# BurntSushi/aho-corasick

Measured on NVIDIA H100. Metric: haystack_scan_throughput, higher is better.
Workload: dtype u8

## Files before the change

aho-corasick_b200/csrc/acb_prefilter.cu:

```cuda
#include "acb_device.cuh"
#ifndef ACB_PTX_HEADER
#define ACB_PTX_HEADER "acb_ptx.cuh"
#endif
#include ACB_PTX_HEADER

#include <cstdio>
#include <cstdlib>
#include <type_traits>

#include <cub/device/device_scan.cuh>
#include <cub/device/device_select.cuh>

namespace acb {
namespace {

enum : int { kGeomNarrow = 0, kGeomWide = 1 };
template <int GEOM> struct PfGeom {
  static constexpr int kThreads = GEOM == kGeomNarrow ? 1024 : 512;
  static constexpr int kWarps = kThreads / 32;
  static constexpr int kGroups = GEOM == kGeomNarrow ? 2 : 4;
  static constexpr int kTile = kGroups * 512;
  static constexpr int kStageBytes = kTile + 16;
  static constexpr int kMinCtas = GEOM == kGeomWide ? 2 : 1;
};
template <bool DENSE> struct PfCfg {
  static constexpr int kSlots = 256;
  static constexpr int kQ2 = DENSE ? 64 : 96;
};

__device__ __forceinline__ uint32_t bloom_hash2(uint32_t x) {
  x ^= x >> 16;
  x *= 0x7feb352du;
  x ^= x >> 15;
  x *= 0x846ca68bu;
  x ^= x >> 16;
  return x;
}

__device__ __forceinline__ uint32_t bloom_hash3(uint32_t x) {
  x ^= x >> 15;
  x *= 0x2c1b3c6du;
  x ^= x >> 12;
  x *= 0x297a2d39u;
  x ^= x >> 15;
  return x;
}

#ifdef ACB_EMULATE
static const uint32_t kWinShift = getenv("ACB_EMU_WINSHIFT") ? (uint32_t)atoi(getenv("ACB_EMU_WINSHIFT")) : 31u;
#else
constexpr uint32_t kWinShift = 31;
#endif

constexpr int kPfStages = 2;

struct Emitter {
  uint64_t* g_keys;
  uint32_t* g_pids;
  unsigned long long* g_counter;
  uint64_t cap;
  __device__ __forceinline__ void emit(uint64_t key, uint32_t pid) {
    const unsigned m = __activemask();
    const int leader = __ffs(m) - 1;
    const int lane = threadIdx.x & 31;
    unsigned long long base = 0;
    if (lane == leader) base = atomicAdd(g_counter, (unsigned long long)__popc(m));
    base = __shfl_sync(m, base, leader);
    const unsigned long long g = base + __popc(m & ((1u << lane) - 1));
    if (g < cap) { g_keys[g] = key; g_pids[g] = pid; }
  }
};

__device__ __forceinline__ uint32_t anchor_lookup(const DfaDev& d, const PrefilterLaunch& p, uint64_t s) {
  if (s + d.amap_k > p.span_end) return 0;
  const uintptr_t a = reinterpret_cast<uintptr_t>(p.hay + s);
  const uintptr_t lo_edge = reinterpret_cast<uintptr_t>(p.hay), hi_edge = lo_edge + p.hay_len;
  const uintptr_t wa = a & ~uintptr_t(3);
  uint32_t key;
  if (wa >= lo_edge && wa + ((a & 3) ? 8 : 4) <= hi_edge) {
    const uint32_t* w = reinterpret_cast<const uint32_t*>(wa);
    const uint32_t lo = __ldg(w);
    const uint32_t hi = (a & 3) ? __ldg(w + 1) : 0u;
    key = __funnelshift_r(lo, hi, (uint32_t)(a & 3) * 8) & d.amap_kmask;
  } else {
    key = 0;
    for (uint32_t i = 0; i < d.amap_k; ++i) key |= (uint32_t)__ldg(p.hay + s + i) << (8 * i);
  }
  uint32_t slot = bloom_hash3(key) >> d.amap_shift;
  for (;;) {
    const uint2 e = __ldg(d.amap + slot);
    if (e.y == 0 || e.x == key) return e.y;
    slot = (slot + 1) & d.amap_mask;
  }
}

__device__ __forceinline__ uint32_t anchor_lookup_key(const DfaDev& d, uint32_t key) {
  uint32_t slot = bloom_hash3(key) >> d.amap_shift;
  for (;;) {
    const uint2 e = __ldg(d.amap + slot);
    if (e.y == 0 || e.x == key) return e.y;
    slot = (slot + 1) & d.amap_mask;
  }
}

template <int MODE>
__device__ __forceinline__ void verify_from(const DfaDev& d, const PrefilterLaunch& p, const uint8_t* s_cls,
                                            uint64_t s, uint32_t sid, uint32_t j, Emitter& em) {
  const uint8_t* __restrict__ hay = p.hay;
  const uint32_t* __restrict__ trans = d.trans;
  uint64_t pos = s + j;
  uint32_t best_pid = 0, best_len = 0;
  bool entered = j != 0;
  for (;;) {
    if (!entered) {
      if (pos >= p.span_end) break;
      const uint32_t b = __ldg(hay + pos);
      sid = __ldg(trans + sid + s_cls[b]);
      ++j;
      ++pos;
      if (sid == 0) break;
      if (__ldg(d.depth16 + (sid >> d.stride2)) != j) break;
    }
    entered = false;
    if (sid <= d.max_match_id) {
      const uint32_t row = sid >> d.stride2;
      const uint32_t lo = __ldg(d.match_offsets + row - 2), hi = __ldg(d.match_offsets + row - 1);
      if (MODE == 0) {
        for (uint32_t i = lo; i < hi; ++i) {
          const uint32_t pid = __ldg(d.match_pids + i);
          if (__ldg(d.pattern_lens + pid) != j) break;
          if (p.first_only && i > lo) break;
          const uint64_t tie = ((uint64_t)(d.max_pattern_len - j) << p.dup_shift) | (uint64_t)(i - lo);
          em.emit(((pos - p.span_start) << kTieBits) | tie, pid);
        }
      } else {
        const uint32_t pid = __ldg(d.match_pids + lo);
        if (__ldg(d.pattern_lens + pid) == j) { best_pid = pid; best_len = j; }
      }
    }
  }
  if (MODE == 1 && best_len) em.emit(((s - p.span_start) << kTieBits) | best_len, best_pid);
}

template <int MODE>
__device__ __forceinline__ void verify_at(const DfaDev& d, const PrefilterLaunch& p, const uint8_t* s_cls,
                                          uint64_t s, Emitter& em) {
  if (d.amap != nullptr) {
    const uint32_t sid = anchor_lookup(d, p, s);
    if (sid != 0) verify_from<MODE>(d, p, s_cls, s, sid, d.amap_k, em);
  } else {
    verify_from<MODE>(d, p, s_cls, s, d.start_unanchored_id, 0, em);
  }
}

template <int GEOM> struct PfBloom {
  static constexpr uint32_t kLogBits = GEOM == kGeomWide ? 17 : 20;
  static constexpr uint32_t kShift = 35 - kLogBits;
};

template <uint32_t SHIFT>
__device__ __forceinline__ bool bloom_test(const uint32_t* s_bitmap, uint32_t h) {
  const uint32_t byte = reinterpret_cast<const uint8_t*>(s_bitmap)[h >> SHIFT];
  const uint32_t rep = byte * 0x01010101u;
  return (__funnelshift_r(rep, rep, h) & 1u) != 0;
}

template <int MODE, bool MASKED, bool DENSE, int STRIDE, int GEOM, int DYN = 0>
__global__ void __launch_bounds__(PfGeom<GEOM>::kThreads, PfGeom<GEOM>::kMinCtas)
prefilter_kernel(DfaDev d, PrefilterLaunch p) {
  static_assert(STRIDE == 1 || STRIDE == 2, "fingerprint stride");
  static_assert(GEOM == kGeomNarrow || STRIDE == 2, "the 2 KiB tile needs the stride-2 first stage (32 hit bits per lane)");
  constexpr bool ANCH = DENSE;
  constexpr int kPfThreads = PfGeom<GEOM>::kThreads;
  constexpr int kPfWarps = PfGeom<GEOM>::kWarps;
  constexpr int kPfTile = PfGeom<GEOM>::kTile;
  constexpr int kPfStageBytes = PfGeom<GEOM>::kStageBytes;
  constexpr int kGroups = PfGeom<GEOM>::kGroups;
  constexpr int kPfSlots = PfCfg<DENSE>::kSlots;
  constexpr int kSlotsAlloc = kPfSlots;
  constexpr int kPfQ2 = PfCfg<ANCH>::kQ2;
  constexpr uint32_t kBloomShift = PfBloom<GEOM>::kShift;
  using Q2Entry = typename std::conditional<ANCH, uint2, uint32_t>::type;
  ACB_DYNAMIC_SMEM(smem_raw);
  unsigned char* s_ring = smem_raw;
  uint64_t* s_bars = reinterpret_cast<uint64_t*>(s_ring + kPfWarps * kPfStages * kPfStageBytes);
  uint32_t* s_tile_of = reinterpret_cast<uint32_t*>(s_bars + kPfWarps * kPfStages);
  uint32_t* s_next_tile = s_tile_of + kPfWarps * kPfStages;
  Q2Entry* s_queue2 = reinterpret_cast<Q2Entry*>(s_next_tile + 4);
  uint16_t* s_slots = reinterpret_cast<uint16_t*>(s_queue2 + kPfWarps * kPfQ2);
  uint32_t* s_bitmap = reinterpret_cast<uint32_t*>(s_slots + kPfWarps * kSlotsAlloc);
  __shared__ uint8_t s_cls[256];

  const int tid = threadIdx.x;
  const int lane = tid & 31;
  const int warp = tid >> 5;
  const uint32_t bitmap_words = p.brute ? 0u : (1u << (p.log_bits - 5));
  for (uint32_t i = tid; i < bitmap_words; i += kPfThreads) s_bitmap[i] = p.bitmap[i];
  if (tid < 256) s_cls[tid] = d.classes[tid];
  if (tid < kPfWarps * kPfStages) ptx::mbar_init(ptx::smem_addr(&s_bars[tid]), 1);
  if (tid == 0) {
    *reinterpret_cast<uint64_t*>(s_next_tile) = DYN == 2 ? (uint64_t)blockIdx.x << 32 : 0ull;
    s_next_tile[2] = 0xFFFFFFFEu;
  }
  ptx::mbar_init_fence();
  ptx::fence_proxy_async();
  __syncthreads();

  Emitter em{p.keys, p.pids, p.counter, p.cap};
  unsigned long long cand_total = 0;

  if (blockIdx.x == 0) {
    const uint64_t tail_lo = (p.region_hi > p.region_lo && !p.brute) ? p.region_hi - (STRIDE - 1) : p.region_hi;
    const uint64_t head_n = p.region_lo - p.scan_lo;
    const uint64_t tail_n = p.scan_hi > tail_lo ? p.scan_hi - tail_lo : 0;
    for (uint64_t i = tid; i < head_n + tail_n; i += kPfThreads) {
      const uint64_t s = i < head_n ? p.scan_lo + i : tail_lo + (i - head_n);
      verify_at<MODE>(d, p, s_cls, s, em);
    }
  }

  const uint64_t n_blocks16 = (p.region_hi - p.region_lo) >> 4;
  const uint64_t per_cta = (n_blocks16 + gridDim.x - 1) / gridDim.x;
  const uint64_t b0 = (uint64_t)blockIdx.x * per_cta;
  const uint64_t b1 = min(b0 + per_cta, n_blocks16);
  const uint64_t split_lo = p.region_lo + (b0 << 4);
  const uint64_t split_hi = b0 < b1 ? p.region_lo + (b1 << 4) : split_lo;

  if (p.brute) {
    for (uint64_t s = split_lo + tid; s < split_hi; s += kPfThreads) verify_at<MODE>(d, p, s_cls, s, em);
    if (tid == 0 && split_hi > split_lo) atomicAdd(p.counter + 1, (unsigned long long)(split_hi - split_lo));
    return;
  }
  constexpr bool whole = DYN == 2;
  const uint64_t chunk_lo = whole ? p.region_lo : split_lo;
  const uint64_t chunk_hi = whole ? p.region_hi : split_hi;

  const uint32_t kmask = p.kmask, fold = p.fold, mult = p.mult;
  const uint32_t fold1 = p.fold & 0x00FFFFFFu;
  const uint32_t mult8 = p.mult3 << p.key_shift;
  const uint64_t chunk_base = chunk_lo - (uint64_t)(STRIDE - 1);
  const uint32_t rel_bias = (uint32_t)(STRIDE - 1);
  const uint8_t* s_bytes = reinterpret_cast<const uint8_t*>(s_bitmap);
  unsigned char* ring = s_ring + warp * (kPfStages * kPfStageBytes);
  uint64_t* bars = s_bars + warp * kPfStages;
  uint16_t* slots = s_slots + warp * kSlotsAlloc;
  Q2Entry* q2 = s_queue2 + warp * kPfQ2;
  uint32_t q2len = 0;
  uint32_t q2win = 0;

  auto drain2 = [&]() {
    __syncwarp();
    const uint64_t win_base = chunk_base + ((uint64_t)q2win << kWinShift);
    for (uint32_t i = lane; i < q2len; i += 32) {
      if constexpr (ANCH) {
        const uint2 e = q2[i];
        if (e.y != 0) verify_from<MODE>(d, p, s_cls, win_base + e.x, e.y, d.amap_k, em);
        else verify_at<MODE>(d, p, s_cls, win_base + e.x, em);
      } else {
        verify_at<MODE>(d, p, s_cls, win_base + q2[i], em);
      }
    }
    cand_total += q2len;
    q2len = 0;
    __syncwarp();
  };

  const uint64_t chunk_bytes = chunk_hi - chunk_lo;
  const uint32_t n_tiles = (uint32_t)((chunk_bytes + kPfTile - 1) / kPfTile);
  const uint32_t last_valid = n_tiles ? (uint32_t)(chunk_bytes - (uint64_t)(n_tiles - 1) * kPfTile) : 0;
  const bool use_windows = (chunk_bytes >> kWinShift) != 0;
  uint32_t bar0 = ptx::smem_addr(bars), ring0 = ptx::smem_addr(ring), lane0 = ring0 + (uint32_t)lane * 16u;
  ptx::keep_in_registers(bar0, ring0, lane0);
  const uint8_t* chunk_src = p.hay + chunk_lo;
  auto issue = [&](uint32_t t, uint32_t stage) {
    const uint32_t bytes = (t + 1 < n_tiles ? (uint32_t)kPfTile : last_valid) + 16;
    const uint32_t bar = bar0 + stage * 8, dst = ring0 + stage * kPfStageBytes;
    ptx::mbar_arrive_expect_tx(bar, bytes);
    ptx::tma_load_1d(dst, chunk_src + (uint64_t)t * kPfTile, bytes, bar);
  };
  constexpr uint32_t kDrawBatch = 4, kSuper = 256;
  static_assert(kSuper % (2 * kDrawBatch) == 0, "batches never straddle a super-tile or its half-way mark");
  uint32_t* tile_of = s_tile_of + warp * kPfStages;
  const uint32_t draw_a = ptx::smem_addr(s_next_tile), next_a = draw_a + 8;
  const uint32_t n_super = (n_tiles + kSuper - 1) / kSuper;
  constexpr uint64_t kNoMore = 0xFFFFFFFFull << 32;
  constexpr uint32_t kUnpublished = 0xFFFFFFFEu, kNone = 0xFFFFFFFFu;
  uint32_t batch_next = 0, batch_left = 0;
  bool exhausted = false;
  unsigned long long pend_g = 0;
  bool have_pend = false;
  auto publish = [&]() {
    if (have_pend) {
      ptx::sts32_volatile(next_a, pend_g < n_super ? (uint32_t)pend_g : kNone);
      have_pend = false;
    }
  };
  auto draw = [&](uint32_t stage) {
    if constexpr (DYN == 1) {
      if (batch_left == 0) {
        batch_next = ptx::atoms_add(draw_a, kDrawBatch);
        batch_left = kDrawBatch;
      }
      const uint32_t t = batch_next++;
      --batch_left;
      tile_of[stage] = t;
      if (t < n_tiles) issue(t, stage);
      return;
    }
    publish();
    while (batch_left == 0 && !exhausted) {
      const uint64_t v = ptx::atoms_add64(draw_a, kDrawBatch);
      const uint32_t sup = (uint32_t)(v >> 32), off = (uint32_t)v;
      if (sup == kNone) { exhausted = true; break; }
      if (off == kSuper / 2) { pend_g = atomicAdd(p.counter + 2, 1ull) + gridDim.x; have_pend = true; }
      if (off < kSuper) { batch_next = sup * kSuper + off; batch_left = kDrawBatch; break; }
      if (off == kSuper) {
        uint32_t g;
        while ((g = ptx::lds32_volatile(next_a)) == kUnpublished) {}
        ptx::sts32_volatile(next_a, kUnpublished);
        if (g != kNone) {
          ptx::atoms_exch64(draw_a, ((uint64_t)g << 32) | kDrawBatch);
          batch_next = g * kSuper;
          batch_left = kDrawBatch;
        } else {
          ptx::atoms_exch64(draw_a, kNoMore);
          exhausted = true;
        }
        break;
      }
      while ((uint32_t)(ptx::lds64_volatile(draw_a) >> 32) == sup) {}
    }
    uint32_t t = n_tiles;
    if (!exhausted) { t = batch_next++; --batch_left; }
    tile_of[stage] = t;
    if (t < n_tiles) issue(t, stage);
  };
  if (lane == 0) {
    if constexpr (DYN) {
      draw(0);
      draw(1);
    } else {
      if ((uint32_t)warp < n_tiles) issue((uint32_t)warp, 0);
      if ((uint32_t)warp + kPfWarps < n_tiles) issue((uint32_t)warp + kPfWarps, 1);
    }
  }
  __syncwarp();
  constexpr int kBitsPerGroup = 16 / STRIDE;
  constexpr int kHitBits = kGroups * kBitsPerGroup;
  for (uint32_t it = 0;; ++it) {
    const uint32_t stage = it & 1;
    const uint32_t parity = (it >> 1) & 1;
    uint32_t t;
    if constexpr (DYN) t = *reinterpret_cast<volatile uint32_t*>(tile_of + stage);
    else t = (uint32_t)warp + it * (uint32_t)kPfWarps;
    if (t >= n_tiles) break;
    const uint64_t wbase = chunk_lo + (uint64_t)t * kPfTile;
    uint32_t win = 0;
    if (use_windows) {
      win = (uint32_t)(((uint64_t)t * kPfTile) >> kWinShift);
      if (win != q2win) {
        if (q2len) drain2();
        q2win = win;
      }
    }
    while (!ptx::mbar_try_wait(bar0 + stage * 8, parity)) {}
    const uint32_t stage_off = stage * (uint32_t)kPfStageBytes;
    const uint32_t tile_a = ring0 + stage_off;
    uint32_t wv[kGroups][5];
#pragma unroll
    for (int g = 0; g < kGroups; ++g) {
      const uint32_t ga = lane0 + stage_off + g * 512;
      const uint4 v = ptx::lds128(ga);
      wv[g][0] = v.x; wv[g][1] = v.y; wv[g][2] = v.z; wv[g][3] = v.w;
      wv[g][4] = ptx::lds32(ga + 16);
    }
    uint32_t mask = 0;
#define ACB_WIN(o, lo, hi) (((o) & 3) ? __funnelshift_r(lo, hi, ((o) & 3) * 8) : (lo))
#define ACB_PROBE(o, lo, hi)                                                                  \
  do {                                                                                        \
    uint32_t gm, h, sel;                                                                      \
    if constexpr (STRIDE == 2) {                                                              \
      gm = MASKED ? (ACB_WIN(o, lo, hi) | fold1) : ACB_WIN(o, lo, hi);                        \
      h = gm * mult8;                                                                         \
      sel = gm;                                                                               \
    } else {                                                                                  \
      gm = MASKED ? ((ACB_WIN(o, lo, hi) | fold) & kmask) : ACB_WIN(o, lo, hi);               \
      h = gm * mult;                                                                          \
      sel = h;                                                                                \
    }                                                                                         \
    if constexpr (DENSE) {                                                                    \
                        \
      const uint32_t ph = __umulhi(gm, mult);                                                  \
      const uint32_t bw = s_bitmap[h >> (kBloomShift + 2)];                                    \
      mask = __funnelshift_r(mask, __funnelshift_r(bw, bw, ph) & __funnelshift_r(bw, bw, ph >> 5), 1); \
    } else {                                                                                  \
      const uint32_t rep = (uint32_t)s_bytes[h >> kBloomShift] * 0x01010101u;                 \
      mask = __funnelshift_r(mask, __funnelshift_r(rep, rep, sel), 1);                        \
    }                                                                                         \
  } while (0)
#pragma unroll
    for (int g = 0; g < kGroups; ++g) {
#pragma unroll
      for (int wi = 0; wi < 4; ++wi) {
        if constexpr (STRIDE == 1) {
          ACB_PROBE(0, wv[g][wi], wv[g][wi + 1]); ACB_PROBE(1, wv[g][wi], wv[g][wi + 1]);
          ACB_PROBE(2, wv[g][wi], wv[g][wi + 1]); ACB_PROBE(3, wv[g][wi], wv[g][wi + 1]);
        } else {
          ACB_PROBE(0, wv[g][wi], wv[g][wi + 1]); ACB_PROBE(2, wv[g][wi], wv[g][wi + 1]);
        }
      }
    }
#undef ACB_PROBE
#undef ACB_WIN
    if constexpr (kHitBits < 32) mask >>= (32 - kHitBits);
    if (t + 1 == n_tiles) {
      uint32_t ok_bits = 0;
#pragma unroll
      for (int g = 0; g < kGroups; ++g)
        if ((uint32_t)(g * 512 + lane * 16) < last_valid) ok_bits |= (uint32_t)((1ull << kBitsPerGroup) - 1) << (g * kBitsPerGroup);
      mask &= ok_bits;
    }
    auto hit_offset = [&](uint32_t b, uint32_t ln) -> uint32_t {
      return (b / kBitsPerGroup) * 512 + ln * 16 + (b % kBitsPerGroup) * STRIDE;
    };
    const uint32_t cnt = __popc(mask);
    const uint32_t lt = (1u << lane) - 1;
    constexpr int kPlanes = DENSE ? 4 : 3;
    uint32_t slot = 0, total = 0;
    constexpr int kSumPlanes = kPlanes;
#pragma unroll
    for (int b = 0; b < kSumPlanes; ++b) {
      const uint32_t bl = __ballot_sync(0xffffffffu, (cnt >> b) & 1u);
      slot += __popc(bl & lt) << b;
      total += __popc(bl) << b;
    }
    if (__any_sync(0xffffffffu, (cnt >> kPlanes) != 0)) total = (uint32_t)kPfSlots + 1;
    if (total) {
      const bool region_first = (whole || blockIdx.x == 0) && t == 0;
      if (total > (uint32_t)kPfSlots) {
        uint32_t nver = 0;
        while (mask) {
          const int b = __ffs(mask) - 1;
          mask &= mask - 1;
          const uint64_t e = wbase + hit_offset((uint32_t)b, (uint32_t)lane);
#pragma unroll
          for (int j = 0; j < STRIDE; ++j)
            if (e >= p.region_lo + j) { verify_at<MODE>(d, p, s_cls, e - j, em); ++nver; }
        }
        cand_total += __reduce_add_sync(0xffffffffu, nver);
      } else {
        {
          uint16_t* sp = slots + slot;
          const uint32_t tag = (uint32_t)lane << 5;
          while (mask) {
            const uint32_t b = (uint32_t)__ffs(mask) - 1;
            mask &= mask - 1;
            *sp++ = (uint16_t)(tag | b);
          }
        }
        __syncwarp();
        const uint32_t wrel = (use_windows ? (uint32_t)((wbase - chunk_lo) - ((uint64_t)win << kWinShift)) : (uint32_t)(wbase - chunk_lo)) + rel_bias;
        const uint32_t n_items = total * STRIDE;
        if constexpr (ANCH) {
          for (uint32_t base = 0; base < n_items; base += 64) {
            uint32_t rel2[2], key2[2], slot2[2], sid2[2];
            bool look[2], pass2[2];
            uint2 ent[2];
#pragma unroll
            for (int u = 0; u < 2; ++u) {
              const uint32_t w = base + 32u * u + lane;
              const uint32_t j = STRIDE == 2 ? (w & 1u) : 0u;
              look[u] = false; pass2[u] = false; rel2[u] = 0; key2[u] = 0; slot2[u] = 0; sid2[u] = 0;
              ent[u] = make_uint2(0, 0);
              if (w < n_items) {
                const uint32_t raw = slots[STRIDE == 2 ? (w >> 1) : w];
                const uint32_t e = hit_offset(raw & 31u, raw >> 5);
                rel2[u] = wrel + e - j;
                if (STRIDE == 2 && e < j) {
                  pass2[u] = !region_first;
                } else if (d.amap == nullptr) {
                  pass2[u] = true;
                } else if (chunk_base + ((uint64_t)win << kWinShift) + rel2[u] + d.amap_k <= p.span_end) {
                  const uint32_t off = e - j;
                  const uint32_t sa = tile_a + (off & ~3u);
                  key2[u] = __funnelshift_r(ptx::lds32(sa), ptx::lds32(sa + 4), (off & 3) * 8) & d.amap_kmask;
                  slot2[u] = bloom_hash3(key2[u]) >> d.amap_shift;
                  look[u] = true;
                }
              }
            }
#pragma unroll
            for (int u = 0; u < 2; ++u)
              if (look[u]) ent[u] = __ldg(d.amap + slot2[u]);
#pragma unroll
            for (int u = 0; u < 2; ++u) {
              if (look[u]) {
                while (ent[u].y != 0 && ent[u].x != key2[u]) {
                  slot2[u] = (slot2[u] + 1) & d.amap_mask;
                  ent[u] = __ldg(d.amap + slot2[u]);
                }
                sid2[u] = ent[u].y;
                pass2[u] = sid2[u] != 0;
              }
              const uint32_t bal = __ballot_sync(0xffffffffu, pass2[u]);
              if (bal) {
                if (pass2[u]) q2[q2len + __popc(bal & lt)] = make_uint2(rel2[u], sid2[u]);
                q2len += __popc(bal);
                if (q2len > (uint32_t)(kPfQ2 - 32)) drain2();
              }
            }
          }
        } else
        for (uint32_t base = 0; base < n_items; base += 32) {
          const uint32_t w = base + lane;
          const uint32_t j = STRIDE == 2 ? (w & 1u) : 0u;
          bool pass = false;
          uint32_t gram_keep = 0, e = 0;
          if (w < n_items) {
            const uint32_t raw = slots[STRIDE == 2 ? (w >> 1) : w];
            e = hit_offset(raw & 31u, raw >> 5);
            if (STRIDE == 2 && e < j) {
              pass = !region_first;
            } else {
              const uint32_t off = e - j;
              const uint32_t sa = tile_a + (off & ~3u);
              uint32_t gram = __funnelshift_r(ptx::lds32(sa), ptx::lds32(sa + 4), (off & 3) * 8);
              if (MASKED) gram = (gram | fold) & kmask;
              if (STRIDE == 2) pass = bloom_test<kBloomShift>(s_bitmap, gram * mult) && bloom_test<kBloomShift>(s_bitmap, bloom_hash2(gram));
              else pass = bloom_test<kBloomShift>(s_bitmap, bloom_hash2(gram));
            }
          }
          const uint32_t bal = __ballot_sync(0xffffffffu, pass);
          if (bal) {
            if (pass) {
              const uint32_t rel = wrel + e - j;
              if constexpr (!ANCH) q2[q2len + __popc(bal & lt)] = rel;
            }
            q2len += __popc(bal);
            if (q2len > (uint32_t)(kPfQ2 - 32)) drain2();
          }
        }
      }
    }
    __syncwarp();
    if (lane == 0) {
      if constexpr (DYN) draw(stage);
      else if (t + 2 * kPfWarps < n_tiles) issue(t + 2 * kPfWarps, stage);
    }
  }
  if constexpr (DYN == 2) { if (lane == 0) publish(); }
  if (q2len) drain2();
  if (lane == 0 && cand_total) atomicAdd(p.counter + 1, cand_total);
}

constexpr int kBsThreads = 512;
constexpr int kBsWarps = kBsThreads / 32;
constexpr int kBsQueue = 128;

template <int MODE>
__global__ void __launch_bounds__(kBsThreads, 2) bytescan_kernel(DfaDev d, PrefilterLaunch p) {
  __shared__ uint8_t s_cls[256];
  __shared__ uint64_t s_q[kBsWarps * kBsQueue];
  const int tid = threadIdx.x, lane = tid & 31, warp = tid >> 5;
  if (tid < 256) s_cls[tid] = d.classes[tid];
  __syncthreads();
  Emitter em{p.keys, p.pids, p.counter, p.cap};
  unsigned long long cand_total = 0;
  if (blockIdx.x == 0) {
    const uint64_t head_n = p.region_lo - p.scan_lo;
    const uint64_t tail_n = p.scan_hi > p.region_hi ? p.scan_hi - p.region_hi : 0;
    for (uint64_t i = tid; i < head_n + tail_n; i += kBsThreads)
      verify_at<MODE>(d, p, s_cls, i < head_n ? p.scan_lo + i : p.region_hi + (i - head_n), em);
  }
  uint64_t* q = s_q + warp * kBsQueue;
  uint32_t qlen = 0;
  auto drain = [&]() {
    __syncwarp();
    for (uint32_t i = lane; i < qlen; i += 32) verify_at<MODE>(d, p, s_cls, q[i], em);
    cand_total += qlen;
    qlen = 0;
    __syncwarp();
  };
  const uint32_t n_needles = p.bs_n;
  const uint32_t max_back = max(p.bs_back[0], max(p.bs_back[1], p.bs_back[2]));
  const uint32_t owned_lanes = max_back ? 31u : 32u;
  const uint64_t step_bytes = (uint64_t)owned_lanes * 16;
  const uint64_t region_bytes = p.region_hi - p.region_lo;
  const uint64_t n_steps = (region_bytes + step_bytes - 1) / step_bytes;
  const uint32_t lt = (1u << lane) - 1;
  const uint64_t load_end = p.region_hi + (max_back ? 16 : 0);
  auto load = [&](uint64_t base) -> uint4 {
    return base < load_end ? ptx::ld_nc_u4(p.hay + base) : make_uint4(0, 0, 0, 0);
  };
  auto process = [&](uint64_t base, const uint4& v) {
    const bool in_range = base < load_end;
    const uint32_t w[4] = {v.x, v.y, v.z, v.w};
    uint32_t zany = 0;
#pragma unroll
    for (int j = 0; j < 3; ++j) {
      if (j >= (int)n_needles) break;
      const uint32_t needle = p.bs_needle[j];
#pragma unroll
      for (int k = 0; k < 4; ++k) {
        const uint32_t x = w[k] ^ needle;
        zany |= (x - 0x01010101u) & ~x & 0x80808080u;
      }
    }
    if (!__any_sync(0xffffffffu, zany != 0 && in_range)) return;
    uint32_t cand = 0;
#pragma unroll
    for (int j = 0; j < 3; ++j) {
      if (j >= (int)n_needles) break;
      const uint32_t needle = p.bs_needle[j];
      uint32_t m = 0;
#pragma unroll
      for (int k = 0; k < 4; ++k) {
        const uint32_t x = w[k] ^ needle;
        const uint32_t z = (x - 0x01010101u) & ~x & 0x80808080u;
        m |= ((((z >> 7) * 0x00204081u) >> 21) & 0xFu) << (4 * k);
      }
      if (!in_range) m = 0;
      const uint32_t back = p.bs_back[j];
      if (back == 0) {
        cand |= m;
      } else {
        const uint32_t both = m | (__shfl_down_sync(0xffffffffu, m, 1) << 16);
        uint32_t smear = both;
        for (uint32_t sft = 1; sft <= back; ++sft) smear |= both >> sft;
        cand |= smear & 0xFFFFu;
      }
    }
    if (lane >= (int)owned_lanes || base >= p.region_hi) cand = 0;
    const uint32_t cnt = __popc(cand);
    if (__any_sync(0xffffffffu, cnt != 0)) {
      uint32_t slot = 0, total = 0;
#pragma unroll
      for (int b = 0; b < 5; ++b) {
        const uint32_t bl = __ballot_sync(0xffffffffu, (cnt >> b) & 1u);
        slot += __popc(bl & lt) << b;
        total += __popc(bl) << b;
      }
      if (qlen + total > (uint32_t)kBsQueue) drain();
      if (total > (uint32_t)kBsQueue) {
        uint32_t c = cand, nver = 0;
        while (c) {
          const int bit = __ffs(c) - 1;
          c &= c - 1;
          verify_at<MODE>(d, p, s_cls, base + bit, em);
          ++nver;
        }
        cand_total += __reduce_add_sync(0xffffffffu, nver);
      } else {
        uint64_t* dst = q + qlen + slot;
        uint32_t c = cand;
        while (c) {
          const int bit = __ffs(c) - 1;
          c &= c - 1;
          *dst++ = base + bit;
        }
        qlen += total;
        if (qlen >= 64) drain();
      }
    }
  };
  const uint64_t stride = (uint64_t)gridDim.x * kBsWarps;
  auto base_of = [&](uint64_t st) { return p.region_lo + st * step_bytes + (uint64_t)lane * 16; };
  uint64_t st = (uint64_t)blockIdx.x * kBsWarps + warp;
  uint4 cur[2], nxt[2];
#pragma unroll
  for (int u = 0; u < 2; ++u) cur[u] = st + u * stride < n_steps ? load(base_of(st + u * stride)) : make_uint4(0, 0, 0, 0);
  for (; st < n_steps; st += 2 * stride) {
#pragma unroll
    for (int u = 0; u < 2; ++u) {
      const uint64_t sn = st + (2 + u) * stride;
      nxt[u] = sn < n_steps ? load(base_of(sn)) : make_uint4(0, 0, 0, 0);
    }
#pragma unroll
    for (int u = 0; u < 2; ++u)
      if (st + u * stride < n_steps) process(base_of(st + u * stride), cur[u]);
    cur[0] = nxt[0];
    cur[1] = nxt[1];
  }
  if (qlen) drain();
  if (lane == 0 && cand_total) atomicAdd(p.counter + 1, cand_total);
}


__device__ __forceinline__ void tuple_span(const ChainLaunch& c, uint64_t i, uint64_t* s, uint64_t* e) {
  const uint64_t key = c.keys[i];
  if (c.mode == 1) {
    *s = key >> kTieBits;
    *e = *s + (key & kTieMask);
  } else {
    *e = key >> kTieBits;
    *s = *e - c.pattern_lens[c.pids[i]];
  }
}

__global__ void chain_ends_kernel(ChainLaunch c) {
  const uint64_t i = (uint64_t)blockIdx.x * blockDim.x + threadIdx.x;
  if (i >= c.n) return;
  uint64_t s, e;
  tuple_span(c, i, &s, &e);
  c.scratch_end[i] = e;
}

__global__ void chain_select_kernel(ChainLaunch c) {
  const uint64_t i = (uint64_t)blockIdx.x * blockDim.x + threadIdx.x;
  if (i >= c.n) return;
  uint64_t s, e;
  tuple_span(c, i, &s, &e);
  if (i > 0 && c.scratch_end[i - 1] > s) return;
  c.flags[i] = 1;
  uint64_t cur_end = e;
  for (uint64_t j = i + 1; j < c.n; ++j) {
    uint64_t sj, ej;
    tuple_span(c, j, &sj, &ej);
    if (c.scratch_end[j - 1] <= sj) break;
    if (sj >= cur_end) { c.flags[j] = 1; cur_end = ej; } else c.flags[j] = 0;
  }
}

struct MaxOp {
  __device__ __forceinline__ uint64_t operator()(uint64_t a, uint64_t b) const { return a > b ? a : b; }
};

}

cudaError_t launch_prefilter(const DfaDev& dfa, const PrefilterLaunch& p, int sm_count, cudaStream_t s) {
  const bool dense = p.dense != 0;
  const int geom = p.stride == 2 ? p.geom : kGeomNarrow;
  if (geom < kGeomNarrow || geom > kGeomWide) return cudaErrorInvalidValue;
  const uint32_t want_log = geom == kGeomWide ? PfBloom<kGeomWide>::kLogBits : PfBloom<kGeomNarrow>::kLogBits;
  if (!p.brute && (p.log_bits != want_log || p.shift != 35 - want_log)) return cudaErrorInvalidValue;
  const size_t bitmap_bytes = p.brute ? 0 : (size_t(1) << (p.log_bits - 3));
  static const int kThreadsOf[2] = {PfGeom<0>::kThreads, PfGeom<1>::kThreads};
  static const int kStageOf[2] = {PfGeom<0>::kStageBytes, PfGeom<1>::kStageBytes};
  static const int kTileOf[2] = {PfGeom<0>::kTile, PfGeom<1>::kTile};
  const int threads = kThreadsOf[geom];
  const int warps = threads / 32;
  const int stage_bytes = kStageOf[geom];
  const int tile = kTileOf[geom];
  const int q2_bytes = dense ? PfCfg<true>::kQ2 * 8 : PfCfg<false>::kQ2 * 4;
  const int slot_bytes = PfCfg<false>::kSlots * 2;
  const size_t smem = size_t(warps) * (kPfStages * stage_bytes + kPfStages * 12 + q2_bytes + slot_bytes) + 16 + bitmap_bytes;
  if (smem > 227 * 1024 - 1024) return cudaErrorInvalidValue;
  const bool masked = p.fold != 0 || p.kmask != 0xFFFFFFFFu;
  using KernT = void (*)(DfaDev, PrefilterLaunch);
#define ACB_PF_ROW(M, K, D)                                                                                 \
  {prefilter_kernel<M, K, false, 1, kGeomNarrow, D>, prefilter_kernel<M, K, true, 1, kGeomNarrow, D>, \
   prefilter_kernel<M, K, false, 2, kGeomNarrow, D>, prefilter_kernel<M, K, false, 2, kGeomWide, D>}
  static const KernT table[2][2][3][4] = {
      {{ACB_PF_ROW(0, false, 0), ACB_PF_ROW(0, false, 1), ACB_PF_ROW(0, false, 2)},
       {ACB_PF_ROW(0, true, 0), ACB_PF_ROW(0, true, 1), ACB_PF_ROW(0, true, 2)}},
      {{ACB_PF_ROW(1, false, 0), ACB_PF_ROW(1, false, 1), ACB_PF_ROW(1, false, 2)},
       {ACB_PF_ROW(1, true, 0), ACB_PF_ROW(1, true, 1), ACB_PF_ROW(1, true, 2)}}};
#undef ACB_PF_ROW
  if (p.dyn > 2) return cudaErrorInvalidValue;
  if (p.stride == 2 && dense) return cudaErrorInvalidValue;
  int variant = dense ? 1 : 0;
  if (p.stride == 2) variant = geom == kGeomWide ? 3 : 2;
  KernT kern = table[p.mode ? 1 : 0][masked ? 1 : 0][p.dyn][variant];
#ifdef ACB_EMULATE
  if (getenv("ACB_EMU_TRACE")) fprintf(stderr, "launch_prefilter variant %d dyn %d threads %d smem %zu\n", variant, (int)p.dyn, threads, smem);
#endif
  cudaError_t e = cudaFuncSetAttribute(kern, cudaFuncAttributeMaxDynamicSharedMemorySize, (int)smem);
  if (e != cudaSuccess) return e;
  int per_sm = 1;
  e = cudaOccupancyMaxActiveBlocksPerMultiprocessor(&per_sm, kern, threads, smem);
  if (e != cudaSuccess) return e;
  if (per_sm < 1) per_sm = 1;
  uint64_t grid = (uint64_t)sm_count * per_sm;
  const uint64_t cta_step = uint64_t(warps) * tile;
  const uint64_t warp_steps = ((p.region_hi - p.region_lo) + cta_step - 1) / cta_step;
  if (grid > warp_steps) grid = warp_steps ? warp_steps : 1;
  ACB_LAUNCH(kern, (unsigned)grid, threads, smem, s, dfa, p);
  return cudaGetLastError();
}

cudaError_t launch_bytescan(const DfaDev& dfa, const PrefilterLaunch& p, int sm_count, cudaStream_t s) {
  if (p.bs_n < 1 || p.bs_n > 3) return cudaErrorInvalidValue;
  for (uint32_t j = 0; j < 3; ++j)
    if (p.bs_back[j] > 15) return cudaErrorInvalidValue;
  uint64_t grid = (uint64_t)sm_count * 2;
  const uint64_t steps = ((p.region_hi - p.region_lo) + 16 * 31 - 1) / (16 * 31);
  const uint64_t ctas = (steps + kBsWarps - 1) / kBsWarps;
  if (grid > ctas) grid = ctas ? ctas : 1;
  if (p.mode) ACB_LAUNCH(bytescan_kernel<1>, (unsigned)grid, kBsThreads, 0, s, dfa, p);
  else ACB_LAUNCH(bytescan_kernel<0>, (unsigned)grid, kBsThreads, 0, s, dfa, p);
  return cudaGetLastError();
}

cudaError_t launch_chain_ends(const ChainLaunch& c, cudaStream_t s) {
  const unsigned blocks = (unsigned)((c.n + 255) / 256);
  ACB_LAUNCH(chain_ends_kernel, blocks, 256, 0, s, c);
  return cudaGetLastError();
}
cudaError_t launch_chain_select(const ChainLaunch& c, cudaStream_t s) {
  const unsigned blocks = (unsigned)((c.n + 255) / 256);
  ACB_LAUNCH(chain_select_kernel, blocks, 256, 0, s, c);
  return cudaGetLastError();
}
cudaError_t scan_max_u64(void* d_temp, size_t& temp_bytes, uint64_t* data, uint64_t n, cudaStream_t s) {
  return cub::DeviceScan::InclusiveScan(d_temp, temp_bytes, data, data, MaxOp(), (int64_t)n, s);
}
cudaError_t select_flagged(void* d_temp, size_t& temp_bytes, const uint64_t* keys_in, const uint32_t* pids_in,
                           const uint8_t* flags, uint64_t* keys_out, uint32_t* pids_out,
                           unsigned long long* d_num_out, uint64_t n, cudaStream_t s) {
  size_t a = 0, b = 0;
  if (d_temp == nullptr) {
    cudaError_t e = cub::DeviceSelect::Flagged(nullptr, a, keys_in, flags, keys_out, d_num_out, (int64_t)n, s);
    if (e != cudaSuccess) return e;
    e = cub::DeviceSelect::Flagged(nullptr, b, pids_in, flags, pids_out, d_num_out, (int64_t)n, s);
    temp_bytes = a > b ? a : b;
    return e;
  }
  cudaError_t e = cub::DeviceSelect::Flagged(d_temp, temp_bytes, keys_in, flags, keys_out, d_num_out, (int64_t)n, s);
  if (e != cudaSuccess) return e;
  return cub::DeviceSelect::Flagged(d_temp, temp_bytes, pids_in, flags, pids_out, d_num_out, (int64_t)n, s);
}

}
```

Before: 1656.

## Use single-stage double-size tiles for narrow stride-2 prefilter warps

```diff
diff --git a/aho-corasick_b200/csrc/acb_prefilter.cu b/aho-corasick_b200/csrc/acb_prefilter.cu
--- a/aho-corasick_b200/csrc/acb_prefilter.cu
+++ b/aho-corasick_b200/csrc/acb_prefilter.cu
@@ -53,6 +53,14 @@
 #endif
 
 constexpr int kPfStages = 2;
+
+template <int GEOM, int STRIDE> struct PfPass {
+  static constexpr bool kPair = STRIDE == 2 && GEOM == kGeomNarrow;
+  static constexpr int kStages = kPair ? 1 : kPfStages;
+  static constexpr int kGroups = PfGeom<GEOM>::kGroups * (kPair ? 2 : 1);
+  static constexpr int kTile = kGroups * 512;
+  static_assert(kStages * (kTile + 16) <= kPfStages * PfGeom<GEOM>::kStageBytes, "a step's tiles fit the warp's ring");
+};
 
 struct Emitter {
   uint64_t* g_keys;
@@ -173,9 +181,11 @@
   constexpr bool ANCH = DENSE;
   constexpr int kPfThreads = PfGeom<GEOM>::kThreads;
   constexpr int kPfWarps = PfGeom<GEOM>::kWarps;
-  constexpr int kPfTile = PfGeom<GEOM>::kTile;
-  constexpr int kPfStageBytes = PfGeom<GEOM>::kStageBytes;
-  constexpr int kGroups = PfGeom<GEOM>::kGroups;
+  constexpr int kRingBytes = kPfStages * PfGeom<GEOM>::kStageBytes;
+  constexpr int kStages = PfPass<GEOM, STRIDE>::kStages;
+  constexpr int kPfTile = PfPass<GEOM, STRIDE>::kTile;
+  constexpr int kPfStageBytes = kPfTile + 16;
+  constexpr int kGroups = PfPass<GEOM, STRIDE>::kGroups;
   constexpr int kPfSlots = PfCfg<DENSE>::kSlots;
   constexpr int kSlotsAlloc = kPfSlots;
   constexpr int kPfQ2 = PfCfg<ANCH>::kQ2;
@@ -183,7 +193,7 @@
   using Q2Entry = typename std::conditional<ANCH, uint2, uint32_t>::type;
   ACB_DYNAMIC_SMEM(smem_raw);
   unsigned char* s_ring = smem_raw;
-  uint64_t* s_bars = reinterpret_cast<uint64_t*>(s_ring + kPfWarps * kPfStages * kPfStageBytes);
+  uint64_t* s_bars = reinterpret_cast<uint64_t*>(s_ring + kPfWarps * kRingBytes);
   uint32_t* s_tile_of = reinterpret_cast<uint32_t*>(s_bars + kPfWarps * kPfStages);
   uint32_t* s_next_tile = s_tile_of + kPfWarps * kPfStages;
   Q2Entry* s_queue2 = reinterpret_cast<Q2Entry*>(s_next_tile + 4);
@@ -241,7 +251,7 @@
   const uint64_t chunk_base = chunk_lo - (uint64_t)(STRIDE - 1);
   const uint32_t rel_bias = (uint32_t)(STRIDE - 1);
   const uint8_t* s_bytes = reinterpret_cast<const uint8_t*>(s_bitmap);
-  unsigned char* ring = s_ring + warp * (kPfStages * kPfStageBytes);
+  unsigned char* ring = s_ring + warp * kRingBytes;
   uint64_t* bars = s_bars + warp * kPfStages;
   uint16_t* slots = s_slots + warp * kSlotsAlloc;
   Q2Entry* q2 = s_queue2 + warp * kPfQ2;
@@ -338,18 +348,18 @@
   if (lane == 0) {
     if constexpr (DYN) {
       draw(0);
-      draw(1);
+      if (kStages > 1) draw(1);
     } else {
       if ((uint32_t)warp < n_tiles) issue((uint32_t)warp, 0);
-      if ((uint32_t)warp + kPfWarps < n_tiles) issue((uint32_t)warp + kPfWarps, 1);
+      if (kStages > 1 && (uint32_t)warp + kPfWarps < n_tiles) issue((uint32_t)warp + kPfWarps, 1);
     }
   }
   __syncwarp();
   constexpr int kBitsPerGroup = 16 / STRIDE;
   constexpr int kHitBits = kGroups * kBitsPerGroup;
   for (uint32_t it = 0;; ++it) {
-    const uint32_t stage = it & 1;
-    const uint32_t parity = (it >> 1) & 1;
+    const uint32_t stage = kStages == 1 ? 0u : it & 1;
+    const uint32_t parity = (kStages == 1 ? it : it >> 1) & 1;
     uint32_t t;
     if constexpr (DYN) t = *reinterpret_cast<volatile uint32_t*>(tile_of + stage);
     else t = (uint32_t)warp + it * (uint32_t)kPfWarps;
@@ -545,8 +555,9 @@
     __syncwarp();
     if (lane == 0) {
       if constexpr (DYN) draw(stage);
-      else if (t + 2 * kPfWarps < n_tiles) issue(t + 2 * kPfWarps, stage);
-    }
+      else if (t + kStages * kPfWarps < n_tiles) issue(t + kStages * kPfWarps, stage);
+    }
+    if constexpr (DYN && kStages == 1) __syncwarp();
   }
   if constexpr (DYN == 2) { if (lane == 0) publish(); }
   if (q2len) drain2();
@@ -736,11 +747,11 @@
   const size_t bitmap_bytes = p.brute ? 0 : (size_t(1) << (p.log_bits - 3));
   static const int kThreadsOf[2] = {PfGeom<0>::kThreads, PfGeom<1>::kThreads};
   static const int kStageOf[2] = {PfGeom<0>::kStageBytes, PfGeom<1>::kStageBytes};
-  static const int kTileOf[2] = {PfGeom<0>::kTile, PfGeom<1>::kTile};
   const int threads = kThreadsOf[geom];
   const int warps = threads / 32;
   const int stage_bytes = kStageOf[geom];
-  const int tile = kTileOf[geom];
+  const int tile = geom == kGeomWide ? PfPass<kGeomWide, 2>::kTile
+                   : p.stride == 2 ? PfPass<kGeomNarrow, 2>::kTile : PfPass<kGeomNarrow, 1>::kTile;
   const int q2_bytes = dense ? PfCfg<true>::kQ2 * 8 : PfCfg<false>::kQ2 * 4;
   const int slot_bytes = PfCfg<false>::kSlots * 2;
   const size_t smem = size_t(warps) * (kPfStages * stage_bytes + kPfStages * 12 + q2_bytes + slot_bytes) + 16 + bitmap_bytes;
```

Result: faster. 1813 (median of 6 runs) (+9.5%).
